# hrz2000/CustomNeRF

Measured on AMD Instinct MI355X. Metric: training rays/s, higher is better.
Workload: dtype f16

## Files before the change

### customnerf_amd/csrc/field_bwd_x2.hip

```cpp
#include "field_bwd_common.h"

typedef short x4_s4 __attribute__((__vector_size__(4 * sizeof(short))));
typedef short x4_s2 __attribute__((ext_vector_type(2)));

#define X4_K 1024

struct X4Img { uint32_t c0, c1; };
__device__ __forceinline__ uint32_t x4_img_swz(uint32_t byte_off) { return byte_off ^ (((byte_off >> 9) & 3u) << 6); }
template <int S>
__device__ __forceinline__ cn_h8 x4_frag_T(const unsigned char *layer, X4Img lane_off, int tp, int sp) {
    const uint32_t c = ((sp >> 1) * S + 2 * tp) * 1024 + (16 * (sp & 1)) * 16;
    union { cn_h8 h; x4_s4 s[2]; } f;
    f.s[0] = __builtin_amdgcn_ds_read_tr16_b64_v4i16((x4_s4 __attribute__((address_space(3))) *)(layer + lane_off.c0 + c));
    f.s[1] = __builtin_amdgcn_ds_read_tr16_b64_v4i16((x4_s4 __attribute__((address_space(3))) *)(layer + lane_off.c1 + c));
    return f.h;
}
__device__ __forceinline__ X4Img x4_lane_off_w(uint32_t l, bool natural_cols) {
    const uint32_t G = l >> 4, i = l & 15, rho = i >> 2, q = i & 3;
    const uint32_t hi = natural_cols ? (q >> 1) : (q & 1), j0 = natural_cols ? 4 * (q & 1) : 4 * (q >> 1);
    const uint32_t base = (G & 1) * 1024 + hi * 512 + (4 * (l >> 5) + rho) * 16;
    X4Img o;
    o.c0 = x4_img_swz(base) + j0 * 2;
    o.c1 = x4_img_swz(base + 8 * 16) + j0 * 2;
    return o;
}
__device__ __forceinline__ cn_h8 x4_load_frag(const _Float16 *base, uint32_t t, uint32_t S, uint32_t s, uint32_t lane) {
    return *reinterpret_cast<const cn_h8 *>(reinterpret_cast<const unsigned char *>(base) + (t * S + s) * 1024 + ((lane * 16) ^ ((((s & 1) * 2 + (lane >> 5)) << 6))));
}
__device__ __forceinline__ X4Img x4_lane_off_img(uint32_t l, bool natural_slots) {
    const uint32_t G = l >> 4, i = l & 15, rho = i >> 2, q = i & 3;
    const uint32_t hi = natural_slots ? (q >> 1) : (q & 1), j0 = natural_slots ? 4 * (q & 1) : 4 * (q >> 1);
    const uint32_t base = (G & 1) * 1024 + hi * 512 + (8 * (l >> 5) + rho) * 16;
    X4Img o;
    o.c0 = x4_img_swz(base) + j0 * 2;
    o.c1 = x4_img_swz(base + 4 * 16) + j0 * 2;
    return o;
}
__device__ __forceinline__ cn_h8 x4_frag_img(const unsigned char *img, X4Img lane_off, int u, int kk) {
    const uint32_t c = 2 * u * 1024 + 16 * kk * 16;
    union { cn_h8 h; x4_s4 s[2]; } f;
    f.s[0] = __builtin_amdgcn_ds_read_tr16_b64_v4i16((x4_s4 __attribute__((address_space(3))) *)(img + lane_off.c0 + c));
    f.s[1] = __builtin_amdgcn_ds_read_tr16_b64_v4i16((x4_s4 __attribute__((address_space(3))) *)(img + lane_off.c1 + c));
    return f.h;
}

template <int T, int NS>
__device__ __forceinline__ void x4_gemm(const _Float16 *wf, uint32_t S, uint32_t s0, const cn_h8 *b, uint32_t lane, cn_f16v (&acc)[T]) {
#pragma unroll
    for (int s = 0; s < NS; s++) {
#pragma unroll
        for (int t = 0; t < T; t++) acc[t] = Prec<true>::mfma(x4_load_frag(wf, t, S, s0 + s, lane), b[s], acc[t]);
    }
}

template <int T, int NS, int S>
__device__ __forceinline__ void x4_gemm_T(const unsigned char *layer, X4Img lane_off, const cn_h8 *b, cn_f16v (&acc)[T]) {
#pragma unroll
    for (int s = 0; s < NS; s++) {
#pragma unroll
        for (int t = 0; t < T; t++) acc[t] = Prec<true>::mfma(x4_frag_T<S>(layer, lane_off, t, s), b[s], acc[t]);
    }
}

__device__ __forceinline__ uint32_t x4_cvt_pk(float a, float b) {
    const cn_h2 v = {(_Float16)a, (_Float16)b};
    return __builtin_bit_cast(uint32_t, v);
}
__device__ __forceinline__ uint32_t x4_pk_relu(uint32_t v) {
    uint32_t r;
    asm("v_pk_max_i16 %0, %1, 0" : "=v"(r) : "v"(v));
    return r;
}
__device__ __forceinline__ uint32_t x4_pk_posmask(uint32_t act) {
    uint32_t t, m;
    asm("v_pk_sub_i16 %0, 0, %1" : "=v"(t) : "v"(act));
    asm("v_pk_ashrrev_i16 %0, %1, %2" : "=v"(m) : "v"(0x000F000Fu), "v"(t));
    return m;
}
template <bool RELU>
__device__ __forceinline__ void x4_c_to_b(const cn_f16v (&acc)[2], cn_h8 *b) {
#pragma unroll
    for (int u = 0; u < 2; u++) {
#pragma unroll
        for (int sub = 0; sub < 2; sub++) {
            union { cn_h8 h; uint32_t w[4]; } f;
#pragma unroll
            for (int j = 0; j < 4; j++) {
                const uint32_t v = x4_cvt_pk(acc[u][8 * sub + 2 * j], acc[u][8 * sub + 2 * j + 1]);
                f.w[j] = RELU ? x4_pk_relu(v) : v;
            }
            b[u * 2 + sub] = f.h;
        }
    }
}
__device__ __forceinline__ void x4_c_to_b_masked(const cn_f16v (&acc)[2], const cn_h8 *act, cn_h8 *b) {
#pragma unroll
    for (int u = 0; u < 2; u++) {
#pragma unroll
        for (int sub = 0; sub < 2; sub++) {
            union { cn_h8 h; uint32_t w[4]; } f, a;
            a.h = act[u * 2 + sub];
#pragma unroll
            for (int j = 0; j < 4; j++) f.w[j] = x4_cvt_pk(acc[u][8 * sub + 2 * j], acc[u][8 * sub + 2 * j + 1]) & x4_pk_posmask(a.w[j]);
            b[u * 2 + sub] = f.h;
        }
    }
}

__device__ __forceinline__ void x4_barrier() {
    asm volatile("s_waitcnt lgkmcnt(0)\n\ts_barrier" ::: "memory");
}

template <int SENC>
__device__ __forceinline__ void x4_enc_request(const void *__restrict__ enc, uint32_t P_, uint32_t L, uint32_t p, uint32_t hi, cn_h8 (&b)[SENC]) {
    const uint32_t *e = reinterpret_cast<const uint32_t *>(enc) + min(p, P_ - 1);
#pragma unroll
    for (int s = 0; s < SENC; s++) {
        union { cn_h8 h; uint32_t u[4]; } f;
#pragma unroll
        for (int jj = 0; jj < 4; jj++) f.u[jj] = e[(size_t)min(8 * s + 4 * hi + jj, L - 1) * P_];
        b[s] = f.h;
    }
}
template <int SENC>
__device__ __forceinline__ void x4_enc_mask(const cn_h8 (&raw)[SENC], uint32_t L, bool valid, uint32_t hi, cn_h8 (&b)[SENC]) {
#pragma unroll
    for (int s = 0; s < SENC; s++) {
        union { cn_h8 h; uint32_t u[4]; } f;
        f.h = raw[s];
#pragma unroll
        for (int jj = 0; jj < 4; jj++) f.u[jj] = (valid && (8 * s + 4 * hi + jj) < L) ? f.u[jj] : 0u;
        b[s] = f.h;
    }
}

template <int NS>
__device__ __forceinline__ void x4_publish(unsigned char *img, uint32_t lane, const cn_h8 *x) {
#pragma unroll
    for (int s = 0; s < NS; s++) *reinterpret_cast<cn_h8 *>(img + s * 1024 + ((lane * 16) ^ ((((s & 1) * 2 + (lane >> 5)) << 6)))) = x[s];
}
template <int NS>
__device__ __forceinline__ void x4_fetch(const unsigned char *img, uint32_t lane, cn_h8 *x) {
#pragma unroll
    for (int s = 0; s < NS; s++) x[s] = *reinterpret_cast<const cn_h8 *>(img + s * 1024 + ((lane * 16) ^ ((((s & 1) * 2 + (lane >> 5)) << 6))));
}

__device__ __forceinline__ void x4_dw(cn_f16v &acc, const cn_h8 (&z)[2], const cn_h8 (&a)[2]) {
    acc = Prec<true>::mfma(z[0], a[0], acc);
    acc = Prec<true>::mfma(z[1], a[1], acc);
}
__device__ __forceinline__ void x4_load_block(const unsigned char *img, X4Img lane_off, int u, cn_h8 (&f)[2]) {
    f[0] = x4_frag_img(img, lane_off, u, 0);
    f[1] = x4_frag_img(img, lane_off, u, 1);
}
__device__ __forceinline__ void x4_store(float *__restrict__ part, uint32_t dst, uint32_t stride, uint32_t col0, uint32_t M, uint32_t N, uint32_t mt, uint32_t nt,
                                         uint32_t li, uint32_t hi, const cn_f16v &acc) {
    const uint32_t col = 32 * nt + li;
#pragma unroll
    for (int r = 0; r < 16; r++) {
        const uint32_t row = 32 * mt + (uint32_t)fld_rho(r, (int)hi);
        if (row < M && col < N) part[dst + (size_t)row * stride + col0 + col] = acc[r];
    }
}
__device__ __forceinline__ void x4_zero(cn_f16v &a) {
#pragma unroll
    for (int r = 0; r < 16; r++) a[r] = 0.0f;
}

#define X4_T0() const unsigned long long t0_ = (ablate & 32) ? __builtin_readcyclecounter() : 0ull
#define X4_T1() do { if (ablate & 32) { const unsigned long long t1_ = __builtin_readcyclecounter(); x4_barrier(); \
                                        const unsigned long long t2_ = __builtin_readcyclecounter(); tw_ += t1_ - t0_; tb_ += t2_ - t1_; } else x4_barrier(); } while (0)

#define X2_FEA 0
#define X2_Z3 (2 * 4 * X4_K)
#define X2_A (X2_Z3 + 2 * 4 * X4_K)
#define X2_A_X0 0
#define X2_A_H1 (2 * X4_K)
#define X2_A_H2 (6 * X4_K)
#define X2_A_Z2 (10 * X4_K)
#define X2_A_Z1 (14 * X4_K)
#define X2_B (X2_A + 18 * X4_K)
#define X2_B_HD 0
#define X2_B_HR (4 * X4_K)
#define X2_B_DIR (8 * X4_K)
#define X2_B_ZR (10 * X4_K)
#define X2_B_ZD (14 * X4_K)
#define X2_B_BRO (18 * X4_K)
#define X2_B_BDO (20 * X4_K)
#define X2_PAIR_BYTES (X2_B + 22 * X4_K)

template <int NGEO, bool SKIP>
__global__ void __launch_bounds__(FLD_THREADS) k_field_bwd_x2(const void *__restrict__ enc, const float *__restrict__ xyz, const float *__restrict__ dirs,
                                                              uint32_t dir_group, uint32_t P_, FieldDims dm, const float *__restrict__ pnet,
                                                              const float *__restrict__ pden, const float *__restrict__ prgb,
                                                              const float *__restrict__ g_sigma, const float *__restrict__ g_rgbc,
                                                              void *__restrict__ grad_enc, float *__restrict__ partials, uint32_t ablate_arg,
                                                              const uint8_t *__restrict__ tile_live, const void *__restrict__ wimg) {
#ifdef CNERF_TUNING
    const uint32_t ablate = ablate_arg;
#else
    constexpr uint32_t ablate = 0;
    (void)ablate_arg;
#endif
    constexpr bool H = true;
    constexpr int SENC = 2;
    using PR = Prec<H>;
    using frag_t = typename PR::frag_t;
    using elem_t = typename PR::elem_t;
    __shared__ __attribute__((aligned(16))) elem_t x2_w[FLD_HID * (32 + 3 * FLD_HID + (FLD_HID + FLD_DIR)) + 2 * 32 * FLD_HID];
    extern __shared__ __attribute__((aligned(16))) unsigned char fld_lds[];
    elem_t *wl = x2_w;
    const FieldLds lo = fld_lds_layout<H>(dm);
    const FfOff po = ff_offsets(dm);

    constexpr uint32_t S64 = FLD_HID / PR::KS, SDIR = FLD_DIR / PR::KS, SR0 = S64 + SDIR;
    const uint32_t in_r0 = FLD_HID + FLD_DIR;
    const float *n0 = pnet, *n1 = pnet + FLD_HID * dm.enc_pad;
    const float *n2 = n1 + (NGEO == 2 ? FLD_HID * FLD_HID : 0);
    const float *d0 = pden, *dO = pden + FLD_HID * FLD_HID;
    const float *r0 = prgb, *rO = prgb + FLD_HID * in_r0;

    if (wimg) {
        const uint4 *src = reinterpret_cast<const uint4 *>(wimg);
        uint4 *dst = reinterpret_cast<uint4 *>(wl);
        for (uint32_t c = threadIdx.x; c < lo.off[7] / 8; c += FLD_THREADS) dst[c ^ (((c >> 5) & 3u) << 2)] = src[c];
    } else
    for (int rep = 0; rep < ((ablate & 64) ? 2 : 1); rep++) {
    fld_stage_layer<H, 0, true>(wl + lo.off[0], n0, FLD_HID, dm.enc_pad, 2, SENC, dm.enc_pad, threadIdx.x, blockDim.x);
    if (NGEO == 2) fld_stage_layer<H, 1, true>(wl + lo.off[1], n1, FLD_HID, FLD_HID, 2, S64, FLD_HID, threadIdx.x, blockDim.x);
    fld_stage_layer<H, 1, true>(wl + lo.off[2], n2, FLD_HID, FLD_HID, 2, S64, FLD_HID, threadIdx.x, blockDim.x);
    fld_stage_layer<H, 1, true>(wl + lo.off[3], d0, FLD_HID, FLD_HID, 2, S64, FLD_HID, threadIdx.x, blockDim.x);
    fld_stage_layer<H, 1, true>(wl + lo.off[4], dO, 16, FLD_HID, 1, S64, FLD_HID, threadIdx.x, blockDim.x);
    fld_stage_layer<H, 2, true>(wl + lo.off[5], r0, FLD_HID, in_r0, 2, SR0, in_r0, threadIdx.x, blockDim.x);
    fld_stage_layer<H, 1, true>(wl + lo.off[6], rO, 16, FLD_HID, 1, S64, FLD_HID, threadIdx.x, blockDim.x);
    if (ablate & 64) __syncthreads();
    }
    for (uint32_t i = threadIdx.x; i < 2 * 2 * (X4_K / 4); i += FLD_THREADS) {
        const uint32_t pr_ = i / (2 * (X4_K / 4)), w = i % (2 * (X4_K / 4));
        const uint32_t which = w / (X4_K / 4), k = w % (X4_K / 4);
        reinterpret_cast<uint32_t *>(fld_lds + pr_ * X2_PAIR_BYTES + X2_B + (which ? X2_B_BDO : X2_B_BRO) + X4_K)[k] = 0u;
    }
    __syncthreads();

    const uint32_t lane = threadIdx.x & 63, li = lane & 31, hi = lane >> 5;
    const uint32_t wave = __builtin_amdgcn_readfirstlane(threadIdx.x >> 6);
    const uint32_t pair = wave >> 1, role = wave & 1;
    unsigned char *xch = fld_lds + pair * X2_PAIR_BYTES;
    const unsigned char *wb = reinterpret_cast<const unsigned char *>(x2_w);
    [[maybe_unused]] unsigned long long tw_ = 0, tb_ = 0;
    const uint32_t n_tiles = (P_ + FLD_TILE - 1) / FLD_TILE;
    const uint32_t G = gridDim.x * 2, gp = blockIdx.x * 2 + pair;
    const uint32_t n_iter = (n_tiles + G - 1) / G;
    auto tile_at = [&](uint32_t p) { return 2 * (p * gridDim.x + (blockIdx.x + p * 97u) % gridDim.x) + pair; };
    constexpr uint32_t END = 0xFFFFFFFFu;
    struct LiveIt { uint32_t base; uint64_t m; };
    auto pair_mask = [&](uint32_t base, bool fill) -> uint64_t {
        const uint32_t ph = base + lane;
        uint32_t f = 0;
        if (ph < n_iter) {
            if (SKIP) {
                const uint32_t t0 = tile_at(ph) - pair;
                if (t0 < n_tiles) f = tile_live[t0];
                if (t0 + 1 < n_tiles) f |= tile_live[t0 + 1];
            } else {
                f = 1;
            }
        }
        const uint64_t m = __ballot(f != 0);
        if (SKIP && fill) {
            const uint32_t nv = min(64u, n_iter - base);
            uint64_t dead = ~m & (nv == 64 ? ~0ull : (1ull << nv) - 1);
            while (dead) {
                const uint32_t tile = tile_at(base + (uint32_t)__builtin_ctzll(dead));
                dead &= dead - 1;
                const uint32_t row = tile * FLD_TILE + li;
                if (row < P_) {
#pragma unroll
                    for (int r = 0; r < 16; r += 2) {
                        const uint32_t level = (uint32_t)fld_rho(r, (int)hi) >> 1;
                        if (level < dm.L) reinterpret_cast<uint32_t *>(grad_enc)[(size_t)level * P_ + row] = 0u;
                    }
                }
            }
        }
        return m;
    };
    auto it_next = [&](LiveIt &it, bool fill) -> uint32_t {
        while (it.m == 0) {
            if (it.base + 64 >= n_iter) return END;
            it.base += 64;
            it.m = pair_mask(it.base, fill);
        }
        const uint32_t b = (uint32_t)__builtin_ctzll(it.m);
        it.m &= it.m - 1;
        return it.base + b;
    };
    float *part = partials + (size_t)gp * po.total;
    const uint32_t off_n0 = lo.off[0] * 2, off_n1 = lo.off[1] * 2, off_n2 = lo.off[2] * 2, off_d0 = lo.off[3] * 2, off_dO = lo.off[4] * 2,
                   off_r0 = lo.off[5] * 2, off_rO = lo.off[6] * 2;
    const X4Img lw = x4_lane_off_w(lane, false), lwn = x4_lane_off_w(lane, true);
    const X4Img lc = x4_lane_off_img(lane, false), ln = x4_lane_off_img(lane, true);

    if (role == 0) {
        cn_f16v wn2[2][2], wn1[2][2], wn0[2];
#pragma unroll
        for (int a = 0; a < 2; a++) {
            x4_zero(wn0[a]);
#pragma unroll
            for (int b = 0; b < 2; b++) { x4_zero(wn2[a][b]); x4_zero(wn1[a][b]); }
        }
        struct ASet { frag_t x0[SENC], h1[4], h2[4]; uint32_t p; bool v, live; };
        ASet S0, S1;
#pragma unroll
        for (int s = 0; s < SENC; s++) S0.x0[s] = S1.x0[s] = PR::zero();
#pragma unroll
        for (int s = 0; s < 4; s++) S0.h1[s] = S1.h1[s] = S0.h2[s] = S1.h2[s] = PR::zero();
        S0.p = S1.p = 0; S0.v = S1.v = false; S0.live = S1.live = false;
        frag_t N0[SENC], N1[SENC];
        LiveIt it;
        it.base = 0; it.m = pair_mask(0, true);
        uint32_t pk = it_next(it, true);
        uint32_t kend = pk == END ? 0u : END;
        x4_enc_request<SENC>(enc, P_, dm.L, (pk == END ? 0u : tile_at(pk)) * FLD_TILE + li, hi, N0);
#pragma unroll
        for (int s = 0; s < SENC; s++) N1[s] = PR::zero();
        unsigned char *my = xch + X2_A;
        auto phase = [&](uint32_t k, ASet &S, frag_t (&xcur)[SENC], frag_t (&xnext)[SENC]) __attribute__((always_inline)) {
            X4_T0();
            asm volatile("" ::: "memory");
            const uint32_t pn = pk == END ? END : it_next(it, true);
            if (pn == END && kend == END) kend = k + 1;
            x4_enc_request<SENC>(enc, P_, dm.L, (pn == END ? 0u : tile_at(pn)) * FLD_TILE + li, hi, xnext);
            if (!(ablate & 1) && S.live) {
                const unsigned char *z3i = xch + X2_Z3 + (k & 1) * 4 * X4_K;
                frag_t z3[4];
                x4_fetch<4>(z3i, lane, z3);
                x4_publish<SENC>(my + X2_A_X0, lane, S.x0);
                x4_publish<4>(my + X2_A_H1, lane, S.h1);
                if (NGEO == 2) x4_publish<4>(my + X2_A_H2, lane, S.h2);
                cn_f16v acc[2];
                fld_zero(acc);
                x4_gemm_T<2, S64, S64>(wb + off_n2, lw, z3, acc);
                {
                    const unsigned char *hl = my + ((NGEO == 2) ? X2_A_H2 : X2_A_H1);
                    cn_h8 z[2][2], a[2][2];
                    x4_load_block(z3i, lc, 0, z[0]); x4_load_block(z3i, lc, 1, z[1]);
                    x4_load_block(hl, lc, 0, a[0]); x4_load_block(hl, lc, 1, a[1]);
                    x4_dw(wn2[0][0], z[0], a[0]); x4_dw(wn2[0][1], z[0], a[1]); x4_dw(wn2[1][0], z[1], a[0]); x4_dw(wn2[1][1], z[1], a[1]);
                }
                frag_t z1[4];
                if (NGEO == 2) {
                    frag_t z2[4];
                    x4_c_to_b_masked(acc, S.h2, z2);
                    x4_publish<4>(my + X2_A_Z2, lane, z2);
                    fld_zero(acc);
                    x4_gemm_T<2, S64, S64>(wb + off_n1, lw, z2, acc);
                    cn_h8 z[2][2], a[2][2];
                    x4_load_block(my + X2_A_Z2, lc, 0, z[0]); x4_load_block(my + X2_A_Z2, lc, 1, z[1]);
                    x4_load_block(my + X2_A_H1, lc, 0, a[0]); x4_load_block(my + X2_A_H1, lc, 1, a[1]);
                    x4_dw(wn1[0][0], z[0], a[0]); x4_dw(wn1[0][1], z[0], a[1]); x4_dw(wn1[1][0], z[1], a[0]); x4_dw(wn1[1][1], z[1], a[1]);
                }
                x4_c_to_b_masked(acc, S.h1, z1);
                x4_publish<4>(my + X2_A_Z1, lane, z1);
                cn_f16v denc[1];
                fld_zero(denc);
                x4_gemm_T<1, S64, SENC>(wb + off_n0, lwn, z1, denc);
                {
                    cn_h8 z[2][2], a[2];
                    x4_load_block(my + X2_A_Z1, lc, 0, z[0]); x4_load_block(my + X2_A_Z1, lc, 1, z[1]);
                    x4_load_block(my + X2_A_X0, ln, 0, a);
                    x4_dw(wn0[0], z[0], a); x4_dw(wn0[1], z[1], a);
                }
                if (S.v) {
#pragma unroll
                    for (int r = 0; r < 16; r += 2) {
                        const uint32_t level = (uint32_t)fld_rho(r, (int)hi) >> 1;
                        if (level < dm.L) {
                            union { cn_h2 h; uint32_t u; } v;
                            v.h = cn_h2{(_Float16)denc[0][r], (_Float16)denc[0][r + 1]};
                            reinterpret_cast<uint32_t *>(grad_enc)[(size_t)level * P_ + S.p] = v.u;
                        }
                    }
                }
            }
            if (pk != END && !(ablate & 2)) {
                const uint32_t tile = tile_at(pk);
                S.p = tile * FLD_TILE + li;
                S.v = S.p < P_;
                S.live = tile < n_tiles;
            } else {
                S.live = false; S.v = false;
            }
            if (S.live) {
                x4_enc_mask<SENC>(xcur, dm.L, S.v, hi, S.x0);
                cn_f16v acc[2];
                fld_zero(acc);
                x4_gemm<2, SENC>(wl + lo.off[0], SENC, 0, S.x0, lane, acc);
                x4_c_to_b<true>(acc, S.h1);
                if (NGEO == 2) {
                    fld_zero(acc);
                    x4_gemm<2, S64>(wl + lo.off[1], S64, 0, S.h1, lane, acc);
                    x4_c_to_b<true>(acc, S.h2);
                }
                frag_t fea[4];
                fld_zero(acc);
                x4_gemm<2, S64>(wl + lo.off[2], S64, 0, (NGEO == 2) ? S.h2 : S.h1, lane, acc);
                x4_c_to_b<false>(acc, fea);
                x4_publish<4>(xch + X2_FEA + (k & 1) * 4 * X4_K, lane, fea);
            }
            pk = pn;
            X4_T1();
        };
        for (uint32_t k = 0; kend == END || k < kend + 2; k += 2) {
            phase(k, S0, N0, N1);
            phase(k + 1, S1, N1, N0);
        }
#pragma unroll
        for (int a = 0; a < 2; a++) {
            x4_store(part, po.n0, dm.enc_pad, 0, 64, dm.enc_pad, a, 0, li, hi, wn0[a]);
#pragma unroll
            for (int b = 0; b < 2; b++) {
                x4_store(part, po.n2, 64, 0, 64, 64, a, b, li, hi, wn2[a][b]);
                if (NGEO == 2) x4_store(part, po.n1, 64, 0, 64, 64, a, b, li, hi, wn1[a][b]);
            }
        }
    } else {
        cn_f16v wro[2], wrd[2], wrf[2][2], wdo[2], wd0[2][2];
#pragma unroll
        for (int a = 0; a < 2; a++) {
            x4_zero(wro[a]); x4_zero(wrd[a]); x4_zero(wdo[a]);
#pragma unroll
            for (int b = 0; b < 2; b++) { x4_zero(wrf[a][b]); x4_zero(wd0[a][b]); }
        }
        struct BIn { float x, y, z, gs, dx, dy, dz; float4 gc; uint32_t tile; };
        auto load_in = [&](uint32_t window) __attribute__((always_inline)) {
            BIn r;
            r.tile = window == END ? END : tile_at(window);
            const uint32_t p = min((window == END ? 0u : r.tile) * FLD_TILE + li, P_ - 1);
            r.x = xyz[(size_t)p * 3]; r.y = xyz[(size_t)p * 3 + 1]; r.z = xyz[(size_t)p * 3 + 2];
            r.gs = g_sigma[p];
            r.gc = *reinterpret_cast<const float4 *>(g_rgbc + (size_t)p * 4);
            const float *dp = dirs + (size_t)(p / dir_group) * 3;
            r.dx = dp[0]; r.dy = dp[1]; r.dz = dp[2];
            return r;
        };
        LiveIt it;
        it.base = 0; it.m = pair_mask(0, false);
        uint32_t pk = it_next(it, false);
        uint32_t kend = pk == END ? 0u : END;
        BIn I0 = load_in(pk), I1 = I0;
        unsigned char *my = xch + X2_B;
        const bool dir_uniform = (dir_group % FLD_TILE) == 0;
        auto phase = [&](uint32_t k, const BIn &cur, BIn &nxt) __attribute__((always_inline)) {
            X4_T0();
            asm volatile("" ::: "memory");
            if (k >= 1) {
                if (pk != END) pk = it_next(it, false);
                if (pk == END && kend == END) kend = k;
                nxt = load_in(pk);
            }
            if (k >= 1 && !(ablate & 4) && cur.tile < n_tiles) {
                const uint32_t i = k - 1;
                const uint32_t tile = cur.tile;
                const bool valid = tile * FLD_TILE + li < P_;
                const unsigned char *fe = xch + X2_FEA + (i & 1) * 4 * X4_K;
                frag_t fea[4], dfr[SDIR];
                x4_fetch<4>(fe, lane, fea);
                if (dir_uniform) fld_dir_frags_uniform(cur.dx, cur.dy, cur.dz, lane, hi, my + X2_B_ZD, dfr);
                else fld_dir_frags_from<H>(cur.dx, cur.dy, cur.dz, valid, hi, dfr);
                x4_publish<SDIR>(my + X2_B_DIR, lane, dfr);
                cn_f16v acc[2], out[1];
                frag_t hd[4], hr[4];
                fld_zero(acc);
                x4_gemm<2, S64>(wl + lo.off[3], S64, 0, fea, lane, acc);
                x4_c_to_b<true>(acc, hd);
                x4_publish<4>(my + X2_B_HD, lane, hd);
                fld_zero(out);
                x4_gemm<1, S64>(wl + lo.off[4], S64, 0, hd, lane, out);
                const float raw = (float)(_Float16)out[0][0];
                fld_zero(acc);
                x4_gemm<2, S64>(wl + lo.off[5], SR0, 0, fea, lane, acc);
                x4_gemm<2, SDIR>(wl + lo.off[5], SR0, S64, dfr, lane, acc);
                x4_c_to_b<true>(acc, hr);
                x4_publish<4>(my + X2_B_HR, lane, hr);
                fld_zero(out);
                x4_gemm<1, S64>(wl + lo.off[6], S64, 0, hr, lane, out);
                frag_t bro[1], bdo[1];
                {
                    cn_h8 f = PR::zero(), g = PR::zero();
                    if (valid && hi == 0) {
                        const float x = cur.x, y = cur.y, z = cur.z;
                        const float gg = 5.0f * __expf(-(x * x + y * y + z * z) * (1.0f / 0.08f));
                        g[0] = (_Float16)(cur.gs * __expf(fminf(fmaxf(raw + gg, -15.0f), 15.0f)));
                        const float gcv[4] = {cur.gc.x, cur.gc.y, cur.gc.z, cur.gc.w};
#pragma unroll
                        for (int k = 0; k < 4; k++) {
                            const float sg = (float)(_Float16)__builtin_amdgcn_rcpf(1.0f + __expf(-out[0][k]));
                            f[k] = (_Float16)((k < (int)dm.n_rgb_out) ? gcv[k] * sg * (1.0f - sg) : 0.0f);
                        }
                    }
                    bro[0] = f; bdo[0] = g;
                }
                x4_publish<1>(my + X2_B_BRO, lane, bro);
                x4_publish<1>(my + X2_B_BDO, lane, bdo);
                cn_f16v dfea[2];
                fld_zero(dfea);
                {
                    frag_t zr[4];
                    fld_zero(acc);
                    x4_gemm_T<2, 1, S64>(wb + off_rO, lw, bro, acc);
                    x4_c_to_b_masked(acc, hr, zr);
                    x4_publish<4>(my + X2_B_ZR, lane, zr);
                    x4_gemm_T<2, S64, SR0>(wb + off_r0, lw, zr, dfea);
                }
                cn_h8 fa[2][2];
                x4_load_block(fe, lc, 0, fa[0]); x4_load_block(fe, lc, 1, fa[1]);
                {
                    cn_h8 zo[2], z[2][2], a[2][2], d[2];
                    x4_load_block(my + X2_B_BRO, lc, 0, zo);
                    x4_load_block(my + X2_B_HR, lc, 0, a[0]); x4_load_block(my + X2_B_HR, lc, 1, a[1]);
                    x4_dw(wro[0], zo, a[0]); x4_dw(wro[1], zo, a[1]);
                    x4_load_block(my + X2_B_ZR, lc, 0, z[0]); x4_load_block(my + X2_B_ZR, lc, 1, z[1]);
                    x4_load_block(my + X2_B_DIR, ln, 0, d);
                    x4_dw(wrd[0], z[0], d); x4_dw(wrd[1], z[1], d);
                    x4_dw(wrf[0][0], z[0], fa[0]); x4_dw(wrf[0][1], z[0], fa[1]); x4_dw(wrf[1][0], z[1], fa[0]); x4_dw(wrf[1][1], z[1], fa[1]);
                }
                {
                    frag_t zd[4];
                    fld_zero(acc);
                    x4_gemm_T<2, 1, S64>(wb + off_dO, lw, bdo, acc);
                    x4_c_to_b_masked(acc, hd, zd);
                    x4_publish<4>(my + X2_B_ZD, lane, zd);
                    x4_gemm_T<2, S64, S64>(wb + off_d0, lw, zd, dfea);
                }
                {
                    cn_h8 zo[2], z[2][2], a[2][2];
                    x4_load_block(my + X2_B_BDO, lc, 0, zo);
                    x4_load_block(my + X2_B_HD, lc, 0, a[0]); x4_load_block(my + X2_B_HD, lc, 1, a[1]);
                    x4_dw(wdo[0], zo, a[0]); x4_dw(wdo[1], zo, a[1]);
                    x4_load_block(my + X2_B_ZD, lc, 0, z[0]); x4_load_block(my + X2_B_ZD, lc, 1, z[1]);
                    x4_dw(wd0[0][0], z[0], fa[0]); x4_dw(wd0[0][1], z[0], fa[1]); x4_dw(wd0[1][0], z[1], fa[0]); x4_dw(wd0[1][1], z[1], fa[1]);
                }
                frag_t z3[4];
                x4_c_to_b<false>(dfea, z3);
                x4_publish<4>(xch + X2_Z3 + (i & 1) * 4 * X4_K, lane, z3);
            }
            X4_T1();
        };
        for (uint32_t k = 0; kend == END || k < kend + 2; k += 2) {
            phase(k, I1, I0);
            phase(k + 1, I0, I1);
        }
#pragma unroll
        for (int b = 0; b < 2; b++) {
            x4_store(part, po.rO, 64, 0, dm.n_rgb_out, 64, 0, b, li, hi, wro[b]);
            x4_store(part, po.dO, 64, 0, 1, 64, 0, b, li, hi, wdo[b]);
        }
        for (uint32_t i = dm.n_rgb_out * 64 + lane; i < 16 * 64; i += 64) part[po.rO + i] = 0.0f;
        for (uint32_t i = 64 + lane; i < 16 * 64; i += 64) part[po.dO + i] = 0.0f;
        for (uint32_t i = lane; i < 64 * (96 - FLD_NDIR - 64); i += 64) {
            const uint32_t row = i / (96 - FLD_NDIR - 64), col = FLD_NDIR + 64 + i % (96 - FLD_NDIR - 64);
            part[po.r0 + row * 96 + col] = 0.0f;
        }
#pragma unroll
        for (int a = 0; a < 2; a++) {
            x4_store(part, po.r0, 96, 0, 64, FLD_NDIR, a, 0, li, hi, wrd[a]);
#pragma unroll
            for (int b = 0; b < 2; b++) {
                x4_store(part, po.r0, 96, FLD_NDIR, 64, 64, a, b, li, hi, wrf[a][b]);
                x4_store(part, po.d0, 64, 0, 64, 64, a, b, li, hi, wd0[a][b]);
            }
        }
    }
#ifdef CNERF_TUNING
    if ((ablate & 32) && lane == 0) {
        unsigned long long *tt = reinterpret_cast<unsigned long long *>(partials + (size_t)510 * po.total) + ((size_t)blockIdx.x * 4 + wave) * 2;
        tt[0] = tw_; tt[1] = tb_;
    }
#endif
}

bool x2_eligible(const FieldDims &dm) {
    static const int on = cn_tune_env("CNERF_FIELD_X2_BWD", 1);
    return on && dm.enc_pad == 32 && (dm.n_hidden_geo == 1 || dm.n_hidden_geo == 2);
}

int x2_launch(const void *enc, const float *xyz, const float *dirs, uint32_t dir_group, uint32_t P_, const FieldDims &dm, const float *pnet, const float *pden,
              const float *prgb, const float *g_sigma, const float *g_rgbc, void *grad_enc, float *g_net, float *g_den, float *g_rgb, void *workspace,
              uint32_t max_partials, const uint8_t *tile_live, hipStream_t st, const void *wimg) {
    const FieldLds lo = fld_lds_layout<true>(dm);
    if (lo.off[7] > FLD_HID * (32 + 3 * FLD_HID + (FLD_HID + FLD_DIR)) + 2 * 32 * FLD_HID) return CNERF_EINVAL;
    const uint32_t lds_bytes = 2 * X2_PAIR_BYTES;
    const uint32_t n_tiles = cn_div_up(P_, FLD_TILE);
    uint32_t blocks = cn_div_up(n_tiles, 2);
    if (blocks > max_partials / 2) blocks = max_partials / 2;
    if (blocks > 256) blocks = 256;
    const FfOff po = ff_offsets(dm);
    float *partials = reinterpret_cast<float *>(workspace);
    static const int ablate = cn_tune_env("CNERF_X2_ABLATE", 0);
    if ((ablate & 32) && blocks > 255) blocks = 255;
#define X2_LAUNCH(KERN)                                                                                                                    \
    {                                                                                                                                      \
        auto kern = KERN;                                                                                                                  \
        (void)hipFuncSetAttribute(reinterpret_cast<const void *>(kern), hipFuncAttributeMaxDynamicSharedMemorySize, lds_bytes);            \
        hipLaunchKernelGGL(kern, dim3(blocks), dim3(FLD_THREADS), lds_bytes, st, enc, xyz, dirs, dir_group, P_, dm, pnet, pden, prgb, g_sigma, g_rgbc, \
                           grad_enc, partials, (uint32_t)ablate, tile_live, wimg);                                                             \
    }
    cn_stage(4, st);
    if (tile_live) {
        if (dm.n_hidden_geo == 2) X2_LAUNCH((k_field_bwd_x2<2, true>)) else X2_LAUNCH((k_field_bwd_x2<1, true>))
    } else {
        if (dm.n_hidden_geo == 2) X2_LAUNCH((k_field_bwd_x2<2, false>)) else X2_LAUNCH((k_field_bwd_x2<1, false>))
    }
    cn_stage(5, st);
    int rc = cn_launch_status();
    if (rc) return rc;
    ff_reduce_partials(partials, blocks * 2, po.total, po.d0, po.r0 - po.d0, g_net, g_den, g_rgb, st);
    cn_stage(6, st);
    return cn_launch_status();
}
```

Measured before the change: 8.392 million.

## Prefetch transposed weight fragments and interleave dW MFMAs with LDS loads

The backward field kernel now loads transposed weight fragments into registers ahead of each GEMM. The weight-gradient MFMAs for the previous layer are interleaved with those loads, and sched_barrier pins keep the compiler from undoing the order. Activations for the next set (x0, h1, h2) are published to shared memory at the end of the current phase instead of at the start of their own, taking that store off the critical path. The aim is to hide LDS latency behind matrix-core work, at the cost of higher register pressure and possible occupancy loss.

```diff
diff --git a/customnerf_amd/csrc/field_bwd_x2.hip b/customnerf_amd/csrc/field_bwd_x2.hip
--- a/customnerf_amd/csrc/field_bwd_x2.hip
+++ b/customnerf_amd/csrc/field_bwd_x2.hip
@@ -61,6 +61,24 @@
         for (int t = 0; t < T; t++) acc[t] = Prec<true>::mfma(x4_frag_T<S>(layer, lane_off, t, s), b[s], acc[t]);
     }
 }
+
+template <int T, int NS, int S>
+__device__ __forceinline__ void x4_frags_T(const unsigned char *layer, X4Img lane_off, cn_h8 (&w)[NS][T]) {
+#pragma unroll
+    for (int s = 0; s < NS; s++) {
+#pragma unroll
+        for (int t = 0; t < T; t++) w[s][t] = x4_frag_T<S>(layer, lane_off, t, s);
+    }
+}
+template <int T, int NS>
+__device__ __forceinline__ void x4_gemm_pre(const cn_h8 (&w)[NS][T], const cn_h8 *b, cn_f16v (&acc)[T]) {
+#pragma unroll
+    for (int s = 0; s < NS; s++) {
+#pragma unroll
+        for (int t = 0; t < T; t++) acc[t] = Prec<true>::mfma(w[s][t], b[s], acc[t]);
+    }
+}
+__device__ __forceinline__ void x4_pin() { __builtin_amdgcn_sched_barrier(0); }
 
 __device__ __forceinline__ uint32_t x4_cvt_pk(float a, float b) {
     const cn_h2 v = {(_Float16)a, (_Float16)b};
@@ -325,7 +343,7 @@
 #pragma unroll
         for (int s = 0; s < SENC; s++) N1[s] = PR::zero();
         unsigned char *my = xch + X2_A;
-        auto phase = [&](uint32_t k, ASet &S, frag_t (&xcur)[SENC], frag_t (&xnext)[SENC]) __attribute__((always_inline)) {
+        auto phase = [&](uint32_t k, ASet &S, const ASet &Snext, frag_t (&xcur)[SENC], frag_t (&xnext)[SENC]) __attribute__((always_inline)) {
             X4_T0();
             asm volatile("" ::: "memory");
             const uint32_t pn = pk == END ? END : it_next(it, true);
@@ -333,44 +351,48 @@
             x4_enc_request<SENC>(enc, P_, dm.L, (pn == END ? 0u : tile_at(pn)) * FLD_TILE + li, hi, xnext);
             if (!(ablate & 1) && S.live) {
                 const unsigned char *z3i = xch + X2_Z3 + (k & 1) * 4 * X4_K;
+                const unsigned char *hl = my + ((NGEO == 2) ? X2_A_H2 : X2_A_H1);
                 frag_t z3[4];
+                cn_h8 w2[S64][2];
+                x4_frags_T<2, S64, S64>(wb + off_n2, lw, w2);
                 x4_fetch<4>(z3i, lane, z3);
-                x4_publish<SENC>(my + X2_A_X0, lane, S.x0);
-                x4_publish<4>(my + X2_A_H1, lane, S.h1);
-                if (NGEO == 2) x4_publish<4>(my + X2_A_H2, lane, S.h2);
+                cn_h8 z[2][2], a[2][2];
+                x4_load_block(z3i, lc, 0, z[0]); x4_load_block(z3i, lc, 1, z[1]);
+                x4_load_block(hl, lc, 0, a[0]); x4_load_block(hl, lc, 1, a[1]);
+                x4_pin();
                 cn_f16v acc[2];
                 fld_zero(acc);
-                x4_gemm_T<2, S64, S64>(wb + off_n2, lw, z3, acc);
-                {
-                    const unsigned char *hl = my + ((NGEO == 2) ? X2_A_H2 : X2_A_H1);
-                    cn_h8 z[2][2], a[2][2];
-                    x4_load_block(z3i, lc, 0, z[0]); x4_load_block(z3i, lc, 1, z[1]);
-                    x4_load_block(hl, lc, 0, a[0]); x4_load_block(hl, lc, 1, a[1]);
+                x4_gemm_pre<2, S64>(w2, z3, acc);
+                frag_t z1[4];
+                cn_h8 w0[S64][1];
+                if (NGEO == 2) {
+                    cn_h8 w1[S64][2];
+                    x4_frags_T<2, S64, S64>(wb + off_n1, lw, w1);
+                    x4_pin();
                     x4_dw(wn2[0][0], z[0], a[0]); x4_dw(wn2[0][1], z[0], a[1]); x4_dw(wn2[1][0], z[1], a[0]); x4_dw(wn2[1][1], z[1], a[1]);
-                }
-                frag_t z1[4];
-                if (NGEO == 2) {
                     frag_t z2[4];
                     x4_c_to_b_masked(acc, S.h2, z2);
                     x4_publish<4>(my + X2_A_Z2, lane, z2);
-                    fld_zero(acc);
-                    x4_gemm_T<2, S64, S64>(wb + off_n1, lw, z2, acc);
-                    cn_h8 z[2][2], a[2][2];
                     x4_load_block(my + X2_A_Z2, lc, 0, z[0]); x4_load_block(my + X2_A_Z2, lc, 1, z[1]);
                     x4_load_block(my + X2_A_H1, lc, 0, a[0]); x4_load_block(my + X2_A_H1, lc, 1, a[1]);
+                    fld_zero(acc);
+                    x4_gemm_pre<2, S64>(w1, z2, acc);
+                    x4_frags_T<1, S64, SENC>(wb + off_n0, lwn, w0);
+                    x4_pin();
                     x4_dw(wn1[0][0], z[0], a[0]); x4_dw(wn1[0][1], z[0], a[1]); x4_dw(wn1[1][0], z[1], a[0]); x4_dw(wn1[1][1], z[1], a[1]);
+                } else {
+                    x4_frags_T<1, S64, SENC>(wb + off_n0, lwn, w0);
+                    x4_pin();
+                    x4_dw(wn2[0][0], z[0], a[0]); x4_dw(wn2[0][1], z[0], a[1]); x4_dw(wn2[1][0], z[1], a[0]); x4_dw(wn2[1][1], z[1], a[1]);
                 }
                 x4_c_to_b_masked(acc, S.h1, z1);
                 x4_publish<4>(my + X2_A_Z1, lane, z1);
+                x4_load_block(my + X2_A_Z1, lc, 0, z[0]); x4_load_block(my + X2_A_Z1, lc, 1, z[1]);
+                x4_load_block(my + X2_A_X0, ln, 0, a[0]);
                 cn_f16v denc[1];
                 fld_zero(denc);
-                x4_gemm_T<1, S64, SENC>(wb + off_n0, lwn, z1, denc);
-                {
-                    cn_h8 z[2][2], a[2];
-                    x4_load_block(my + X2_A_Z1, lc, 0, z[0]); x4_load_block(my + X2_A_Z1, lc, 1, z[1]);
-                    x4_load_block(my + X2_A_X0, ln, 0, a);
-                    x4_dw(wn0[0], z[0], a); x4_dw(wn0[1], z[1], a);
-                }
+                x4_gemm_pre<1, S64>(w0, z1, denc);
+                x4_dw(wn0[0], z[0], a[0]); x4_dw(wn0[1], z[1], a[0]);
                 if (S.v) {
 #pragma unroll
                     for (int r = 0; r < 16; r += 2) {
@@ -408,12 +430,17 @@
                 x4_c_to_b<false>(acc, fea);
                 x4_publish<4>(xch + X2_FEA + (k & 1) * 4 * X4_K, lane, fea);
             }
+            if (!(ablate & 1) && Snext.live) {
+                x4_publish<SENC>(my + X2_A_X0, lane, Snext.x0);
+                x4_publish<4>(my + X2_A_H1, lane, Snext.h1);
+                if (NGEO == 2) x4_publish<4>(my + X2_A_H2, lane, Snext.h2);
+            }
             pk = pn;
             X4_T1();
         };
         for (uint32_t k = 0; kend == END || k < kend + 2; k += 2) {
-            phase(k, S0, N0, N1);
-            phase(k + 1, S1, N1, N0);
+            phase(k, S0, S1, N0, N1);
+            phase(k + 1, S1, S0, N1, N0);
         }
 #pragma unroll
         for (int a = 0; a < 2; a++) {
@@ -505,42 +532,42 @@
                 x4_publish<1>(my + X2_B_BDO, lane, bdo);
                 cn_f16v dfea[2];
                 fld_zero(dfea);
+                cn_h8 fa[2][2];
+                cn_h8 wh[S64][2];
+                cn_h8 zo[2], z[2][2], a[2][2], d[2];
+                fld_zero(acc);
+                x4_gemm_T<2, 1, S64>(wb + off_rO, lw, bro, acc);
+                x4_frags_T<2, S64, SR0>(wb + off_r0, lw, wh);
+                x4_load_block(my + X2_B_BRO, lc, 0, zo);
+                x4_load_block(my + X2_B_HR, lc, 0, a[0]); x4_load_block(my + X2_B_HR, lc, 1, a[1]);
+                x4_pin();
                 {
                     frag_t zr[4];
-                    fld_zero(acc);
-                    x4_gemm_T<2, 1, S64>(wb + off_rO, lw, bro, acc);
                     x4_c_to_b_masked(acc, hr, zr);
                     x4_publish<4>(my + X2_B_ZR, lane, zr);
-                    x4_gemm_T<2, S64, SR0>(wb + off_r0, lw, zr, dfea);
-                }
-                cn_h8 fa[2][2];
-                x4_load_block(fe, lc, 0, fa[0]); x4_load_block(fe, lc, 1, fa[1]);
-                {
-                    cn_h8 zo[2], z[2][2], a[2][2], d[2];
-                    x4_load_block(my + X2_B_BRO, lc, 0, zo);
-                    x4_load_block(my + X2_B_HR, lc, 0, a[0]); x4_load_block(my + X2_B_HR, lc, 1, a[1]);
-                    x4_dw(wro[0], zo, a[0]); x4_dw(wro[1], zo, a[1]);
                     x4_load_block(my + X2_B_ZR, lc, 0, z[0]); x4_load_block(my + X2_B_ZR, lc, 1, z[1]);
                     x4_load_block(my + X2_B_DIR, ln, 0, d);
-                    x4_dw(wrd[0], z[0], d); x4_dw(wrd[1], z[1], d);
-                    x4_dw(wrf[0][0], z[0], fa[0]); x4_dw(wrf[0][1], z[0], fa[1]); x4_dw(wrf[1][0], z[1], fa[0]); x4_dw(wrf[1][1], z[1], fa[1]);
+                    x4_load_block(fe, lc, 0, fa[0]); x4_load_block(fe, lc, 1, fa[1]);
+                    x4_gemm_pre<2, S64>(wh, zr, dfea);
                 }
+                fld_zero(acc);
+                x4_gemm_T<2, 1, S64>(wb + off_dO, lw, bdo, acc);
+                x4_frags_T<2, S64, S64>(wb + off_d0, lw, wh);
+                x4_pin();
+                x4_dw(wro[0], zo, a[0]); x4_dw(wro[1], zo, a[1]);
+                x4_dw(wrd[0], z[0], d); x4_dw(wrd[1], z[1], d);
+                x4_dw(wrf[0][0], z[0], fa[0]); x4_dw(wrf[0][1], z[0], fa[1]); x4_dw(wrf[1][0], z[1], fa[0]); x4_dw(wrf[1][1], z[1], fa[1]);
+                x4_load_block(my + X2_B_BDO, lc, 0, zo);
+                x4_load_block(my + X2_B_HD, lc, 0, a[0]); x4_load_block(my + X2_B_HD, lc, 1, a[1]);
                 {
                     frag_t zd[4];
-                    fld_zero(acc);
-                    x4_gemm_T<2, 1, S64>(wb + off_dO, lw, bdo, acc);
                     x4_c_to_b_masked(acc, hd, zd);
                     x4_publish<4>(my + X2_B_ZD, lane, zd);
-                    x4_gemm_T<2, S64, S64>(wb + off_d0, lw, zd, dfea);
+                    x4_load_block(my + X2_B_ZD, lc, 0, z[0]); x4_load_block(my + X2_B_ZD, lc, 1, z[1]);
+                    x4_gemm_pre<2, S64>(wh, zd, dfea);
                 }
-                {
-                    cn_h8 zo[2], z[2][2], a[2][2];
-                    x4_load_block(my + X2_B_BDO, lc, 0, zo);
-                    x4_load_block(my + X2_B_HD, lc, 0, a[0]); x4_load_block(my + X2_B_HD, lc, 1, a[1]);
-                    x4_dw(wdo[0], zo, a[0]); x4_dw(wdo[1], zo, a[1]);
-                    x4_load_block(my + X2_B_ZD, lc, 0, z[0]); x4_load_block(my + X2_B_ZD, lc, 1, z[1]);
-                    x4_dw(wd0[0][0], z[0], fa[0]); x4_dw(wd0[0][1], z[0], fa[1]); x4_dw(wd0[1][0], z[1], fa[0]); x4_dw(wd0[1][1], z[1], fa[1]);
-                }
+                x4_dw(wdo[0], zo, a[0]); x4_dw(wdo[1], zo, a[1]);
+                x4_dw(wd0[0][0], z[0], fa[0]); x4_dw(wd0[0][1], z[0], fa[1]); x4_dw(wd0[1][0], z[1], fa[0]); x4_dw(wd0[1][1], z[1], fa[1]);
                 frag_t z3[4];
                 x4_c_to_b<false>(dfea, z3);
                 x4_publish<4>(xch + X2_Z3 + (i & 1) * 4 * X4_K, lane, z3);
```

Result: faster. 8.492 million (median of 6 runs) (+1.2%).
